# shichaoy/cube_slam

Hardware: AMD Instinct MI355X
Metric: frames/sec front-end (ORB extract + LSD+LBD lines + cuboid: Canny+DT+sweep+score+select) @640x480 (higher is better)
Workload: dtype f64

## Files before the change

### cube_slam_amd/csrc/lsd.hip

```cpp
#include "common.h"
#include "glibc_sincosf.h"
#include "lsd_regions.h"

#include <cfloat>
#include <chrono>
#include <cmath>
#include <mutex>
#include <omp.h>
#include <vector>

namespace {
constexpr double NOTDEF = -1024.0, PI_ = 3.1415926535897932384626433832795, DEG_TO_RADS = PI_ / 180;
constexpr float NOTDEF_DEG = -1024.0f;
constexpr int KH = 3;

__host__ __device__ inline float fast_atan2f_(float y, float x) {
    const float p1 = 0.9997878412794807f * (float)(180 / PI_), p3 = -0.3258083974640975f * (float)(180 / PI_), p5 = 0.1555786518463281f * (float)(180 / PI_),
                p7 = -0.04432655554792128f * (float)(180 / PI_);
    float ax = fabsf(x), ay = fabsf(y), a, c, c2;
    if (ax >= ay) { c = ay / (ax + (float)DBL_EPSILON); c2 = c * c; a = (((p7 * c2 + p5) * c2 + p3) * c2 + p1) * c; }
    else { c = ax / (ay + (float)DBL_EPSILON); c2 = c * c; a = 90.f - (((p7 * c2 + p5) * c2 + p3) * c2 + p1) * c; }
    if (x < 0) a = 180.f - a;
    if (y < 0) a = 360.f - a;
    return a;
// ... 819 lines not shown
    }
    return status;
}

int cs_lsd_read_filter_lines(cs_ctx *ctx, cs_lsd *l, float length_thres, float *lines, int cap, int *counts, int n_frames) {
    if (!ctx || !l || !lines || !counts || cap < 1 || n_frames < 0 || (size_t)n_frames < l->keylines.size()) return CS_ERR_BAD_ARG;
    int status = CS_OK;
    for (size_t f = 0; f < l->keylines.size(); f++) {
        int n = 0;
        for (const cs_keyline &k : l->keylines[f])
            if (k.octave == 0 && k.lineLength > length_thres) {
                if (n < cap) { float *o = lines + (f * cap + n) * 4; o[0] = k.startPointX * 1.f; o[1] = k.startPointY * 1.f; o[2] = k.endPointX * 1.f; o[3] = k.endPointY * 1.f; }
                n++;
            }
        counts[f] = std::min(n, cap);
        if (n > cap) status = CS_ERR_CAPACITY;
    }
    return status;
}

int cs_lsd_upload(cs_ctx *ctx, cs_lsd *l, const uint8_t *gray, int n_frames, int stride) {
    int r = lsd_upload(ctx, l, gray, n_frames, stride); if (r) return r;
    CS_HIP(ctx, hipStreamSynchronize(ctx->stream));
    return CS_OK;
}

int cs_lsd_geometry(const cs_lsd *l, int *width, int *height, int *max_frames) {
    if (!l) return CS_ERR_BAD_ARG;
    *width = l->W; *height = l->H; *max_frames = l->max_frames;
    return CS_OK;
}
int cs_lsd_set_frames_device(cs_ctx *ctx, cs_lsd *l, const uint8_t *d_gray, int n_frames) {
    if (!ctx || !l || !d_gray || n_frames < 1 || n_frames > l->max_frames) return CS_ERR_BAD_ARG;
    CS_HIP(ctx, hipSetDevice(ctx->device));
    l->n_frames = n_frames; l->have_desc = false;
    CS_HIP(ctx, hipMemcpyAsync(l->d_gray, d_gray, (size_t)n_frames * l->W * l->H, hipMemcpyDeviceToDevice, ctx->stream));
    return CS_OK;
}

int cs_lsd_run(cs_ctx *ctx, cs_lsd *l, int with_lbd) { return lsd_run(ctx, l, with_lbd); }

int cs_lsd_set_region_stage(cs_lsd *l, int stage) {
    if (!l || stage < CS_LSD_REGIONS_AUTO || stage > CS_LSD_REGIONS_BACKLOG) return CS_ERR_BAD_ARG;
    l->region_stage = stage;
    return CS_OK;
}

int cs_lsd_region_stats(cs_ctx *ctx, cs_lsd *l, long out[5]) {
    if (!ctx || !l || !out) return CS_ERR_BAD_ARG;
    for (int i = 0; i < 5; i++) out[i] = l->rg_stats[i];
    return CS_OK;
}

int cs_lsd_read(cs_ctx *ctx, cs_lsd *l, int frame, cs_keyline *out, int cap, int *count, uint8_t *desc) {
    if (!ctx || !l || frame < 0 || frame >= l->n_frames || !count || (int)l->keylines.size() <= frame || (desc && !l->have_desc)) return CS_ERR_BAD_ARG;
    const int n = (int)l->keylines[frame].size();
    *count = n;
    if (!out) return CS_OK;
    if (n > cap) return CS_ERR_CAPACITY;
    memcpy(out, l->keylines[frame].data(), sizeof(cs_keyline) * (size_t)n);
    if (desc && n > 0) memcpy(desc, l->h_desc.p + (size_t)l->line_off[frame] * 32, (size_t)n * 32);
    return CS_OK;
}

int cs_lsd_get_maps(cs_ctx *ctx, cs_lsd *l, int frame, double *scaled, double *modgrad, double *angles, int *sw, int *sh) {
    if (!ctx || !l || frame < 0 || frame >= l->n_frames || !sw || !sh) return CS_ERR_BAD_ARG;
    *sw = l->w; *sh = l->h;
    const size_t n = (size_t)l->w * l->h;
    int r;
    if (scaled) {
        if (!l->scaled_kept) { ctx->err = "cs_lsd_get_maps: the scaled frames are only kept for a batch of the host region stage (a device stage takes their buffer over); modgrad and angles are kept"; return CS_ERR_BAD_ARG; }
        r = cs_d2h(ctx, scaled, l->d_scaled + n * frame, n); if (r) return r;
    }
    if (modgrad) { r = cs_d2h(ctx, modgrad, l->d_mod + n * frame, n); if (r) return r; }
    std::vector<float> deg;
    if (angles) { deg.resize(n); r = cs_d2h(ctx, deg.data(), l->d_ang + n * frame, n); if (r) return r; }
    CS_HIP(ctx, hipStreamSynchronize(ctx->stream));
    if (angles) for (size_t i = 0; i < n; i++) angles[i] = deg[i] == NOTDEF_DEG ? NOTDEF : double(deg[i]) * DEG_TO_RADS;
    return CS_OK;
}

}

int cs_lsd_filter_lines_packed(cs_lsd *l, float length_thres, std::vector<int> &offsets, std::vector<double> &lines) {
    if (!l) return CS_ERR_BAD_ARG;
    offsets.assign(l->keylines.size() + 1, 0); lines.clear();
    for (size_t f = 0; f < l->keylines.size(); f++) {
        for (const cs_keyline &k : l->keylines[f])
            if (k.octave == 0 && k.lineLength > length_thres) { lines.push_back((double)(k.startPointX * 1.f)); lines.push_back((double)(k.startPointY * 1.f)); lines.push_back((double)(k.endPointX * 1.f)); lines.push_back((double)(k.endPointY * 1.f)); }
        offsets[f + 1] = (int)(lines.size() / 4);
    }
    if (lines.empty()) lines.push_back(0.0);
    return CS_OK;
}
void cs_lsd_set_gate(cs_lsd *l, void (*wait)(void *), void (*done)(void *), void *arg) { l->gate_wait = wait; l->gate_done = done; l->gate_arg = arg; }
void cs_lsd_set_shared_gpu(cs_lsd *l, int shared) {
    l->seq_wpb = shared ? 4 : 16;
    l->walk_bg = shared != 0;
}
```

### cube_slam_amd/csrc/lsd_regions.h

```cpp
#pragma once
#include <vector>

#include <hip/hip_runtime.h>
struct cs_ctx;
struct LsdSeq;
int lsd_seq_run(cs_ctx *ctx, LsdSeq **handle, int F, int w, int h, const float *d_ang, const double *d_mod, const int *d_caddr, const float *d_cdeg, const float2 *d_ccs, const int *frame_base,
                std::vector<std::vector<float>> &lines, long *stats, void (*before_seq)(void *), void (*after_seq)(void *), void *gate_arg, int grp_p, int waves_per_workgroup = 16, void *scratch = nullptr,
                size_t scratch_bytes = 0, bool pix_ready = false, bool walk_bg = false);
void lsd_seq_destroy(cs_ctx *ctx, LsdSeq *r);
```

### cube_slam_amd/csrc/lsd_regions.hip

```cpp
#include "common.h"

#include <cfloat>
#include <climits>
#include <cmath>
#include <vector>

#include "lsd_regions.h"
#include "lsd_rg_seq.h"
#include "lsd_rg_wlk.h"

namespace {
constexpr int PAD_PX = 272, PAD_LIST = 272, PAD_RECT = 34;
constexpr double PI_ = rg::PI_, LOG_EPS = 0.0, LSD_SCALE = 0.8;
struct AngMap { int w, h; const float *deg; };

__device__ __forceinline__ double rg_log_gamma_windschitl(double x) { return 0.918938533204673 + (x - 0.5) * log(x) - x + 0.5 * x * log(x * sinh(1 / x) + 1 / (810.0 * pow(x, 6.0))); }
__device__ double rg_log_gamma(double x) {
    if (x > 15.0) return rg_log_gamma_windschitl(x);
    const double q[7] = {75122.6331530, 80916.6278952, 36308.2951477, 8687.24529705, 1168.92649479, 83.8676043424, 2.50662827511};
    double a = (x + 0.5) * log(x + 5.5) - (x + 5.5), b = 0;
    for (int n = 0; n < 7; ++n) { a -= log(x + double(n)); b += q[n] * pow(x, double(n)); }
    return a + log(b);
}
#ifndef RG_IMPROVE_WAVES
#ifndef RG_IMPROVE_WAVES
#define RG_IMPROVE_WAVES 3
#endif
#endif
constexpr int LG_N = 32768;
__global__ void __launch_bounds__(256) lsd_rg_lgamma_table(double *t) { const int i = blockIdx.x * 256 + threadIdx.x; if (i < LG_N) t[i] = i > 0 ? rg_log_gamma(double(i)) : 0.0; }
__device__ __forceinline__ double rg_lgam_int(int x, const double *lgt) { return x < LG_N ? lgt[x] : rg_log_gamma_windschitl(double(x)); }
__device__ double rg_nfa(int n, int k, double p, double LOG_NT, const double *lgt) {
    if (n == 0 || k == 0) return -LOG_NT;
    if (n == k) return -LOG_NT - double(n) * log10(p);
    const double p_term = p / (1 - p);
    const double log1term = (double(n) + 1) - rg_lgam_int(k + 1, lgt) - rg_lgam_int(n - k + 1, lgt) + double(k) * log(p) + double(n - k) * log(1.0 - p);
    double term = exp(log1term);
    const double RELATIVE_ERROR_FACTOR = 100.0;
    auto double_equal = [&](double a, double b) { if (a == b) return true; double abs_diff = fabs(a - b), aa = fabs(a), bb = fabs(b); double abs_max = aa > bb ? aa : bb; if (abs_max < DBL_MIN) abs_max = DBL_MIN; return (abs_diff / abs_max) <= (RELATIVE_ERROR_FACTOR * DBL_EPSILON); };
    if (double_equal(term, 0)) { if (k > n * p) return -log1term / 2.30258509299404568402 - LOG_NT; else return -LOG_NT; }
    double bin_tail = term;
    const double tolerance = 0.1;
    for (int i = k + 1; i <= n; ++i) {
        const double bin_term = double(n - i + 1) / double(i), mult_term = bin_term * p_term;
        term *= mult_term;
        bin_tail += term;
        if (bin_term < 1) {
            const double err = term * ((1 - pow(mult_term, double(n - i + 1))) / (1 - mult_term) - 1);
            if (err < tolerance * fabs(-log10(bin_tail) - LOG_NT) * bin_tail) break;
        }
    }
    return -log10(bin_tail) - LOG_NT;
}
struct RectSpan {
    int mnX, lmY, rmY, flstep, slstep, frstep, srstep, y_first, y_hi;
    __device__ __forceinline__ void set(const rg::Rect &rec, int h) {
        const double half_width = rec.width / 2.0, dyhw = rec.dy * half_width, dxhw = rec.dx * half_width;
        int x0 = int(rec.x1 - dyhw), y0 = int(rec.y1 + dxhw), x1 = int(rec.x2 - dyhw), y1 = int(rec.y2 + dxhw);
        int x2 = int(rec.x2 + dyhw), y2 = int(rec.y2 - dxhw), x3 = int(rec.x1 + dyhw), y3 = int(rec.y1 - dxhw);
        auto cswap = [](int &xa, int &ya, int &xb, int &yb) {
            const bool sw = xa > xb || (xa == xb && ya > yb);
            const int tx = sw ? xb : xa, ty = sw ? yb : ya; xb = sw ? xa : xb; yb = sw ? ya : yb; xa = tx; ya = ty;
        };
        cswap(x0, y0, x1, y1); cswap(x2, y2, x3, y3); cswap(x0, y0, x2, y2); cswap(x1, y1, x3, y3); cswap(x1, y1, x2, y2);
        int mnI = 0, mnY = y0; mnX = x0;
        { bool c = mnY > y1; mnI = c ? 1 : mnI; mnX = c ? x1 : mnX; mnY = c ? y1 : mnY; c = mnY > y2; mnI = c ? 2 : mnI; mnX = c ? x2 : mnX; mnY = c ? y2 : mnY; c = mnY > y3; mnI = c ? 3 : mnI; mnX = c ? x3 : mnX; mnY = c ? y3 : mnY; }
        const int mxY = max(max(y0, y1), max(y2, y3));
        const bool m0 = mnI == 0, le1 = mnI <= 1, is3 = mnI == 3;
        const int lmX = m0 ? x1 : x0; lmY = m0 ? y1 : y0;
        const int iX = le1 ? x2 : x1, iY = le1 ? y2 : y1, jX = is3 ? x2 : x3, jY = is3 ? y2 : y3;
        const bool rj = iX < jX;
        const int rmX = rj ? jX : iX, tlX = rj ? iX : jX; rmY = rj ? jY : iY;
        flstep = (mnY != lmY) ? (mnX - lmX) / (mnY - lmY) : 0;
        slstep = (lmY != tlX) ? (lmX - tlX) / (lmY - tlX) : 0;
        frstep = (mnY != rmY) ? (mnX - rmX) / (mnY - rmY) : 0;
        srstep = (rmY != tlX) ? (rmX - tlX) / (rmY - tlX) : 0;
        y_hi = min(mxY, h - 1); y_first = max(mnY, 0);
    }
    __device__ __forceinline__ bool row(int y, int w, int &lx, int &rx) const {
        const long r = (long)y - y_first;
        auto adv = [&](int first, int second, int ysw) -> long {
            long nf = (long)ysw - y_first; if (nf < 0) nf = 0; if (nf > r) nf = r;
            return nf * first + (r - nf) * second;
        };
        const long lxl = max((long)mnX + adv(flstep, slstep, lmY), 0L), rxl = min((long)mnX + adv(frstep, srstep, rmY), (long)w - 1);
        lx = (int)lxl; rx = (int)rxl;
        return rxl >= lxl;
    }
};
template <int NP> __device__ __forceinline__ void rg_row_count(const float *row, int lx, int rx, int g, int G, double theta, const double *precs, int *alg_pts) {
    for (int x = lx + g; x <= rx; x += 4 * G) {
        float ad[4];
#pragma unroll
        for (int u = 0; u < 4; u++) { const int xx = x + u * G; ad[u] = row[xx <= rx ? xx : rx]; }
#pragma unroll
        for (int u = 0; u < 4; u++) {
            const bool in = x + u * G <= rx && ad[u] != rgs::NOTDEF_F;
            const double a = double(ad[u]) * rg::DEG_TO_RADS;
            const double d = fabs(theta - a), d2 = fabs(d - rg::M_2__PI_), nt = d > rg::M_3_2_PI_ ? d2 : d;
            for (int k = 0; k < NP; k++) alg_pts[k] += in && nt <= precs[k];
        }
    }
}
template <int NP> __device__ void rg_rect_count(const AngMap &F, const rg::Rect &rec, const double *precs, int lane, int &total, int *algs) {
    RectSpan S; S.set(rec, F.h);
    int total_pts = 0, alg_pts[NP];
    for (int k = 0; k < NP; k++) alg_pts[k] = 0;
    const int rows = S.y_hi - S.y_first + 1;
    const int G = (rows > 0 && rows < 64) ? 64 / rows : 1, RB = 64 / G;
    const int lrow = lane / G, g = lane - lrow * G;
    for (int yb = S.y_first; yb <= S.y_hi; yb += RB) {
        const int y = yb + lrow;
        int lx, rx;
        if (y > S.y_hi || lrow >= RB || !S.row(y, F.w, lx, rx)) continue;
        if (g == 0) total_pts += rx - lx + 1;
        rg_row_count<NP>(F.deg + (size_t)y * F.w, lx, rx, g, G, rec.theta, precs, alg_pts);
    }
    for (int off = 32; off > 0; off >>= 1) {
        total_pts += __shfl_xor(total_pts, off);
        for (int k = 0; k < NP; k++) alg_pts[k] += __shfl_xor(alg_pts[k], off);
    }
    total = total_pts;
    for (int k = 0; k < NP; k++) algs[k] = alg_pts[k];
}
__device__ __forceinline__ void rg_rect_count_group(const AngMap &F, const rg::Rect &rec, bool on, int sub, int &tot, int &alg) {
    RectSpan S; S.set(rec, F.h);
    int total_pts = 0, alg_pts[1] = {0};
    if (on)
        for (int y = S.y_first + sub; y <= S.y_hi; y += 8) {
            int lx, rx;
            if (!S.row(y, F.w, lx, rx)) continue;
            total_pts += rx - lx + 1;
            rg_row_count<1>(F.deg + (size_t)y * F.w, lx, rx, 0, 1, rec.theta, &rec.prec, alg_pts);
        }
    for (int off = 1; off < 8; off <<= 1) { total_pts += __shfl_xor(total_pts, off); alg_pts[0] += __shfl_xor(alg_pts[0], off); }
    tot = total_pts; alg = alg_pts[0];
}
__device__ __forceinline__ rg::Rect rg_rect_shfl(const rg::Rect &r, int src) {
    rg::Rect o;
    o.x1 = __shfl(r.x1, src); o.y1 = __shfl(r.y1, src); o.x2 = __shfl(r.x2, src); o.y2 = __shfl(r.y2, src); o.width = __shfl(r.width, src); o.x = __shfl(r.x, src);
    o.y = __shfl(r.y, src); o.theta = __shfl(r.theta, src); o.dx = __shfl(r.dx, src); o.dy = __shfl(r.dy, src); o.prec = __shfl(r.prec, src); o.p = __shfl(r.p, src);
    return o;
}
__device__ double rg_rect_improve(const AngMap &F, rg::Rect &rec, double LOG_NT, int lane, const double *lgt, double log_nfa) {
    const double delta = 0.5, delta_2 = delta / 2.0;
    if (log_nfa > LOG_EPS) return log_nfa;
    const int g = lane >> 3, sub = lane & 7;
    rg::Rect mine;
    int tot = 0, al = 0, cnt = 0;
    auto tolerances = [&]() {
        mine = rec;
        double p = rec.p, precs[5];
#pragma unroll
        for (int n = 0; n < 5; ++n) { p /= 2; precs[n] = p * PI_; if (n <= g) { mine.p = p; mine.prec = precs[n]; } }
        int t, alg[5]; rg_rect_count<5>(F, rec, precs, lane, t, alg);
        tot = t; al = alg[0];
#pragma unroll
        for (int n = 1; n < 5; ++n) if (g == n) al = alg[n];
        cnt = 5;
    };
    auto shrink = [&](int side) {
        mine = rec; cnt = 0;
        double wd = rec.width;
#pragma unroll
        for (int n = 0; n < 5; ++n) if ((wd - delta) >= 0.5) { wd -= delta; cnt++; }
#pragma unroll
        for (int n = 0; n < 5; ++n) if (n <= g && (mine.width - delta) >= 0.5) {
            if (side == 1) { mine.x1 += -mine.dy * delta_2; mine.y1 += mine.dx * delta_2; mine.x2 += -mine.dy * delta_2; mine.y2 += mine.dx * delta_2; }
            else if (side == 2) { mine.x1 -= -mine.dy * delta_2; mine.y1 -= mine.dx * delta_2; mine.x2 -= -mine.dy * delta_2; mine.y2 -= mine.dx * delta_2; }
            mine.width -= delta;
        }
        if (cnt) rg_rect_count_group(F, mine, g < cnt, sub, tot, al);
    };
    auto take_best = [&]() {
        const bool on = g < cnt;
        const double mv = rg_nfa(on ? tot : 0, on ? al : 0, mine.p, LOG_NT, lgt);
        int best = -1;
#pragma unroll
        for (int n = 0; n < 5; ++n) { const double vn = __shfl(mv, 8 * n); if (n < cnt && vn > log_nfa) { log_nfa = vn; best = n; } }
        if (best >= 0) rec = rg_rect_shfl(mine, 8 * best);
    };
    tolerances(); take_best();
    if (log_nfa > LOG_EPS) return log_nfa;
    for (int side = 0; side < 3; side++) {
        shrink(side);
        if (cnt) take_best();
        if (log_nfa > LOG_EPS) return log_nfa;
    }
    if ((rec.width - delta) >= 0.5) { tolerances(); take_best(); }
    return log_nfa;
}

struct SeqParams {
    int F, w, h;
    const int *caddr; const int *frame_base; const float *cdeg; const float2 *ccs; const double *mod; const float *ang;
    float *ang32; float *seed_cs; int *glist; double *rect; size_t rect_stride; int cand_cap; int *cand_cnt; int *status;
    int min_reg_size, list_cap;
    size_t pix_stride;
};
__global__ void __launch_bounds__(256) lsd_rg_fill32(float4 *ang, size_t n4) {
    const size_t i = (size_t)blockIdx.x * 256 + threadIdx.x;
    if (i < n4) ang[i] = make_float4(rgs::NOTDEF_F, rgs::NOTDEF_F, rgs::NOTDEF_F, rgs::NOTDEF_F);
}
__global__ void __launch_bounds__(256) lsd_rg_scatter(SeqParams P) {
    const int f = blockIdx.y, base = P.frame_base[f], ne = P.frame_base[f + 1] - base;
    const int i = blockIdx.x * 256 + threadIdx.x;
    if (i >= ne) return;
    const int q = P.caddr[base + i] & 0x7fffffff;
    const float d = P.cdeg[base + i];
    P.ang32[(size_t)f * P.pix_stride + q] = d;
    const double a = double(d) * rg::DEG_TO_RADS;
    reinterpret_cast<float2 *>(P.seed_cs)[base + i] = make_float2(float(cos(a)), float(sin(a)));
}
__device__ __forceinline__ void lsd_rg_seq_body(const SeqParams &P) {
    const int f = __builtin_amdgcn_readfirstlane(blockIdx.x * (blockDim.x >> 6) + (threadIdx.x >> 6));
    if (f >= P.F) return;
#ifdef RGS_PRIO
    __builtin_amdgcn_s_setprio(RGS_PRIO);
#endif
    const int base = P.frame_base[f];
    rgs::Frame Fr;
    Fr.w = P.w; Fr.h = P.h; Fr.ne = P.frame_base[f + 1] - base;
    Fr.caddr = P.caddr + base; Fr.fre = P.ang32 + (size_t)f * P.pix_stride; Fr.ang = P.ang + (size_t)f * P.w * P.h; Fr.mod = P.mod + (size_t)f * P.w * P.h; Fr.seed_cs = P.seed_cs + 2 * (size_t)base;
    Fr.rect = P.rect + (size_t)f * P.rect_stride; Fr.cand_cap = P.cand_cap; Fr.cand_cnt = P.cand_cnt + f;
    Fr.status = P.status + 4 * f; Fr.min_reg_size = P.min_reg_size; Fr.list_cap = P.list_cap;
    rgs::List L;
    L.glob = P.glist + (size_t)f * rgs::CAP; L.ring[0] = 0;
    rgs::run_frame<rgs::Wave>(Fr, L);
}
#ifdef RGS_WAVES
__global__ void __launch_bounds__(1024) __attribute__((amdgpu_waves_per_eu(RGS_WAVES, RGS_WAVES))) lsd_rg_seq(SeqParams P) { lsd_rg_seq_body(P); }
#else
__global__ void __launch_bounds__(1024) lsd_rg_seq(SeqParams P) { lsd_rg_seq_body(P); }
#endif
constexpr int WLK_SLICES = 8;
struct WlkLaunch { rgl::Batch slice[WLK_SLICES]; int n_slices, waves_per_slice; };
template <int NS> struct WlkMail {
    rgw::Mail<NS> &m; int base;
    __device__ __forceinline__ rgw::Mail<NS> &mail() { return m; }
    __device__ __forceinline__ int slot_of(int l) const { return base + l; }
    __device__ __forceinline__ int ring_size() const { return NS; }
    __device__ __forceinline__ void after_iteration(const rgl::Batch &) {}
};
template <int WK, int NWAVES, int ACC> __global__ void __launch_bounds__(64 * NWAVES) lsd_rg_wlk(WlkLaunch L, int blocks_per_slice) {
    constexpr int NS = WK * 64;
    __shared__ rgw::Mail<NS> mail;
    for (int k = threadIdx.x; k < NS; k += 64 * NWAVES) { mail.slot[k].state = 0; mail.slot[k].fl = 0; mail.ring_id[k] = 0; mail.ring_tick[k] = 0; }
    if (threadIdx.x == 0) { mail.tail = 0; mail.head = 0; mail.walkers_done = 0; }
    __syncthreads();
    const int wv = __builtin_amdgcn_readfirstlane(threadIdx.x >> 6), lane = threadIdx.x & 63;
    const int c = blockIdx.x / blocks_per_slice;
    const rgl::Batch &B = L.slice[c];
    if (wv < WK) {
        const int f0 = ((blockIdx.x - c * blocks_per_slice) * WK + wv) * 64;
        if (f0 < B.F) { WlkMail<NS> mp{mail, wv * 64}; rgw::run_walker<rgl::LWave, ACC>(B, f0, mp); }
        rgw::wg_release();
        if (lane == 0) rgw::lds_add(&mail.walkers_done, 1);
        return;
    }
    for (;;) {
        int t = 0;
        if (lane == 0) t = rgw::lds_add(&mail.head, 1);
        t = __builtin_amdgcn_readfirstlane(t);
        bool quit = false;
        while (__builtin_amdgcn_readfirstlane(rgw::lds_ld(&mail.ring_tick[t % NS])) != t + 1) {
            if (__builtin_amdgcn_readfirstlane(rgw::lds_ld(&mail.walkers_done)) == WK && __builtin_amdgcn_readfirstlane(rgw::lds_ld(&mail.tail)) <= t) { quit = true; break; }
            __builtin_amdgcn_s_sleep(4);
        }
        if (quit) break;
        rgw::serve_ticket<rgs::Wave, NS>(B, mail, t);
    }
}
__global__ void __launch_bounds__(1024) lsd_rg_cand_scan(const int *cand_cnt, int F, int *cand_base) {
    __shared__ int part[1024];
    const int t = threadIdx.x, per = (F + 1023) / 1024;
    int sum = 0;
    for (int k = 0; k < per; k++) { const int f = t * per + k; if (f < F) sum += cand_cnt[f]; }
    part[t] = sum;
    __syncthreads();
    for (int d = 1; d < 1024; d <<= 1) { const int v = t >= d ? part[t - d] : 0; __syncthreads(); part[t] += v; __syncthreads(); }
    int run = part[t] - sum;
    for (int k = 0; k < per; k++) { const int f = t * per + k; if (f < F) { cand_base[f] = run; run += cand_cnt[f]; } }
    if (t == 1023) cand_base[F] = part[1023];
}
__global__ void __launch_bounds__(256) __attribute__((amdgpu_waves_per_eu(RG_IMPROVE_WAVES, RG_IMPROVE_WAVES))) lsd_rg_improve(SeqParams P, const int *cand_base, int n_cand, const double *lgt, float4 *line, uint8_t *has) {
    const int base = (blockIdx.x * 4 + (threadIdx.x >> 6)) * 8, lane = threadIdx.x & 63, grp = lane >> 3, sub = lane & 7;
    if (base >= n_cand) return;
    const double LOG_NT = 5 * (log10(double(P.w)) + log10(double(P.h))) / 2 + log10(11.0);
    auto frame_of = [&](int wv) { int lo = 0, hi = P.F; while (hi - lo > 1) { const int mid = (lo + hi) >> 1; if (cand_base[mid] <= wv) lo = mid; else hi = mid; } return lo; };
    auto load_rect = [&](int wv, int f, rg::Rect &rec) {
        const double *o = P.rect + (size_t)f * P.rect_stride + (size_t)(wv - cand_base[f]) * 12;
        rec.x1 = o[0]; rec.y1 = o[1]; rec.x2 = o[2]; rec.y2 = o[3]; rec.width = o[4]; rec.x = o[5]; rec.y = o[6]; rec.theta = o[7]; rec.dx = o[8]; rec.dy = o[9]; rec.prec = o[10]; rec.p = o[11];
    };
    auto emit = [&](int wv, rg::Rect rec, double log_nfa) {
        const bool ok = log_nfa > LOG_EPS;
        if (ok) {
            rec.x1 += 0.5; rec.y1 += 0.5; rec.x2 += 0.5; rec.y2 += 0.5;
            rec.x1 /= LSD_SCALE; rec.y1 /= LSD_SCALE; rec.x2 /= LSD_SCALE; rec.y2 /= LSD_SCALE;
            line[wv] = make_float4(float(rec.x1), float(rec.y1), float(rec.x2), float(rec.y2));
        }
        has[wv] = ok ? 1 : 0;
    };
    const int mine = base + grp;
    const bool on = mine < n_cand;
    const int f1 = frame_of(on ? mine : n_cand - 1);
    rg::Rect r1;
    load_rect(on ? mine : n_cand - 1, f1, r1);
    double log1;
    {
        RectSpan S; S.set(r1, P.h);
        const float *deg = P.ang + (size_t)f1 * P.w * P.h;
        int tot = 0, alg[1] = {0};
        if (on)
            for (int y = S.y_first + sub; y <= S.y_hi; y += 8) {
                int lx, rx;
                if (!S.row(y, P.w, lx, rx)) continue;
                tot += rx - lx + 1;
                rg_row_count<1>(deg + (size_t)y * P.w, lx, rx, 0, 1, r1.theta, &r1.prec, alg);
            }
        for (int off = 1; off < 8; off <<= 1) { tot += __shfl_xor(tot, off); alg[0] += __shfl_xor(alg[0], off); }
        log1 = rg_nfa(tot, alg[0], r1.p, LOG_NT, lgt);
    }
    if (on && sub == 0 && log1 > LOG_EPS) emit(mine, r1, log1);
    unsigned long long todo = __ballot(on && sub == 0 && !(log1 > LOG_EPS));
    while (todo) {
        const int l = __ffsll((long long)todo) - 1;
        todo &= todo - 1;
        const int wv = base + (l >> 3), f = __shfl(f1, l);
        const double first = __shfl(log1, l);
        rg::Rect rec;
        load_rect(wv, f, rec);
        const AngMap Fr = {P.w, P.h, P.ang + (size_t)f * P.w * P.h};
        const double log_nfa = rg_rect_improve(Fr, rec, LOG_NT, lane, lgt, first);
        if (lane == 0) emit(wv, rec, log_nfa);
    }
}
}

struct LsdSeq {
    int F = 0, w = 0, h = 0; int cand_cap = 0; size_t cap_lines = 0;
    float *d_pix = nullptr; bool pix_borrowed = false;
    rgl::Ent *d_elist = nullptr; float *d_ang32 = nullptr; int *d_order = nullptr;
    int *d_glist = nullptr, *d_cand_cnt = nullptr, *d_cand_base = nullptr, *d_status = nullptr, *d_frame_base = nullptr;
    double *d_rect = nullptr, *d_lgt = nullptr;
    uint8_t *d_has = nullptr;
    float4 *d_line = nullptr;
    cs_pinned<int> h_base, h_status; cs_pinned<uint8_t> h_has; cs_pinned<float4> h_line;
};
void lsd_seq_destroy(cs_ctx *ctx, LsdSeq *r) {
    if (!r) return;
    void *ptrs[] = {r->d_elist, r->d_ang32, r->d_order, r->pix_borrowed ? nullptr : r->d_pix, r->d_glist, r->d_cand_cnt, r->d_cand_base, r->d_status, r->d_frame_base, r->d_rect, r->d_lgt, r->d_has, r->d_line};
    for (void *p : ptrs) cs_dfree(ctx, p);
    r->h_base.release(); r->h_status.release(); r->h_has.release(); r->h_line.release();
    delete r;
}
int lsd_seq_run(cs_ctx *ctx, LsdSeq **handle, int F, int w, int h, const float *d_ang, const double *d_mod, const int *d_caddr, const float *d_cdeg, const float2 *d_ccs, const int *frame_base,
                std::vector<std::vector<float>> &lines, long *stats ,
                void (*before_seq)(void *), void (*after_seq)(void *), void *gate_arg ,
                int grp_p ,
                int waves_per_workgroup ,
                void *scratch, size_t scratch_bytes ,
                bool pix_ready ,
                bool walk_bg ) {
    LsdSeq *r = *handle;
    if (w > 0xffff || h > 0x7fff) return CS_ERR_CAPACITY;
    int max_ne = 0;
    for (int f = 0; f < F; f++) max_ne = std::max(max_ne, frame_base[f + 1] - frame_base[f]);
    int rc;
#define RA_(call) do { rc = (call); if (rc != CS_OK) return rc; } while (0)
    if (!r || r->F < F || r->w != w || r->h != h) {
        lsd_seq_destroy(ctx, r);
        r = new LsdSeq();
        *handle = r;
        r->F = F; r->w = w; r->h = h; r->cand_cap = 4096;
        RA_(cs_dalloc(ctx, &r->d_order, (size_t)F)); RA_(cs_dalloc(ctx, &r->d_rect, (size_t)F * (r->cand_cap * 12 + PAD_RECT)));
        RA_(cs_dalloc(ctx, &r->d_cand_cnt, (size_t)F)); RA_(cs_dalloc(ctx, &r->d_cand_base, (size_t)F + 1));
        RA_(cs_dalloc(ctx, &r->d_status, (size_t)F * 4)); RA_(cs_dalloc(ctx, &r->d_frame_base, (size_t)F + 1));
        RA_(cs_dalloc(ctx, &r->d_lgt, (size_t)LG_N));
        CS_LAUNCH(ctx, "lsd_rg_lgamma_table", lsd_rg_lgamma_table, dim3(LG_N / 256), dim3(256), 0, r->d_lgt);
    }
    RA_(cs_h2d(ctx, r->d_frame_base, frame_base, (size_t)F + 1));
    SeqParams S;
    S.F = F; S.w = w; S.h = h; S.caddr = d_caddr; S.frame_base = r->d_frame_base; S.cdeg = d_cdeg; S.ccs = d_ccs; S.mod = d_mod; S.ang = d_ang;
    S.ang32 = nullptr; S.seed_cs = reinterpret_cast<float *>(const_cast<float2 *>(d_ccs));  S.glist = r->d_glist; S.rect = r->d_rect; S.cand_cap = r->cand_cap; S.cand_cnt = r->d_cand_cnt; S.status = r->d_status;
    const double LOG_NT = 5 * (std::log10(double(w)) + std::log10(double(h))) / 2 + std::log10(11.0);
    S.min_reg_size = int(-LOG_NT / std::log10(rg::ANG_TH / 180));
    S.list_cap = rgs::CAP;
    if (const char *e = getenv("CUBESLAM_LSD_SEQ_CAP")) S.list_cap = std::max(2, std::min(rgs::CAP, atoi(e)));
    if (grp_p != 0 && grp_p != 65) return CS_ERR_BAD_ARG;
    const bool grp = grp_p == 65, pad = grp;
    const size_t rect_stride = (size_t)r->cand_cap * 12 + (pad ? PAD_RECT : 0), list_stride = (size_t)rgl::CAP + (pad ? PAD_LIST : 0);
    S.pix_stride = (size_t)w * h + (pad ? PAD_PX : 0); S.rect_stride = rect_stride;
    const size_t npx = (size_t)F * S.pix_stride;
    if (grp) {
        const size_t head = (size_t)((w + 8 + 3) & ~3);
        if (!r->d_ang32) RA_(cs_dalloc(ctx, &r->d_ang32, head + (size_t)r->F * ((size_t)w * h + PAD_PX) + 16));
        if (!r->d_elist) RA_(cs_dalloc(ctx, &r->d_elist, (size_t)r->F * ((size_t)rgl::CAP + PAD_LIST) + 16));
        S.ang32 = r->d_ang32 + head;
        CS_LAUNCH(ctx, "lsd_rg_fill", lsd_rg_fill32, dim3((unsigned)(((npx + head) / 4 + 1 + 255) / 256)), dim3(256), 0, reinterpret_cast<float4 *>(r->d_ang32), (npx + head) / 4 + 1);
    } else {
        if (!r->d_pix) {
            if (scratch && scratch_bytes >= (size_t)r->F * w * h * sizeof(float) + 64) { r->d_pix = static_cast<float *>(scratch); r->pix_borrowed = true; }
            else RA_(cs_dalloc(ctx, &r->d_pix, (size_t)r->F * w * h + 16));
        }
        if (!r->d_glist) RA_(cs_dalloc(ctx, &r->d_glist, (size_t)r->F * rgs::CAP));
        S.ang32 = r->d_pix; S.glist = r->d_glist;
        if (pix_ready && !r->pix_borrowed) { ctx->err = "lsd_seq_run: the pixel records were announced in the scratch buffer, but the stage does not use it for this batch"; return CS_ERR_BAD_ARG; }
        if (!pix_ready) CS_LAUNCH(ctx, "lsd_rg_fill", lsd_rg_fill32, dim3((unsigned)((npx / 4 + 1 + 255) / 256)), dim3(256), 0, reinterpret_cast<float4 *>(r->d_pix), npx / 4 + 1);
    }
    if (!pix_ready) CS_LAUNCH(ctx, "lsd_rg_scatter", lsd_rg_scatter, dim3((max_ne + 255) / 256, F), dim3(256), 0, S);
    int wpb = std::max(1, std::min(16, waves_per_workgroup));
    RA_(r->h_base.reserve(ctx, (size_t)F + 1)); RA_(r->h_status.reserve(ctx, (size_t)F * 4));
    if (before_seq) before_seq(gate_arg);
    if (grp) {
        const size_t npx = (size_t)w * h, head = (size_t)((w + 8 + 3) & ~3);
        int chunk = (int)std::min<size_t>(4096, 0xffffffffull / (npx * sizeof(double)));
        chunk = std::min(chunk, 1024);
        if (chunk < 1) return CS_ERR_CAPACITY;
        std::vector<int> order((size_t)F);
        for (int c0 = 0; c0 < F; c0 += chunk) {
            const int fc = std::min(chunk, F - c0);
            for (int k = 0; k < fc; k++) order[(size_t)c0 + k] = k;
            std::stable_sort(order.begin() + c0, order.begin() + c0 + fc, [&](int a, int b) { return frame_base[c0 + a + 1] - frame_base[c0 + a] > frame_base[c0 + b + 1] - frame_base[c0 + b]; });
        }
        RA_(cs_h2d(ctx, r->d_order, order.data(), (size_t)F));
        CS_HIP(ctx, hipStreamSynchronize(ctx->stream));
        for (int l0 = 0; l0 < F; l0 += chunk * WLK_SLICES) {
            WlkLaunch L;
            L.n_slices = 0; L.waves_per_slice = (chunk + 63) / 64;
            for (int c0 = l0; c0 < F && L.n_slices < WLK_SLICES; c0 += chunk) {
                const int fc = std::min(chunk, F - c0);
                rgl::Batch &B = L.slice[L.n_slices++];
                B.F = fc; B.w = w; B.h = h; B.npx = (int)npx; B.order = r->d_order + c0; B.ang_stride = (int)S.pix_stride; B.list_stride = (int)list_stride; B.rect_stride = (int)rect_stride; B.ang_head = (int)head;
                B.caddr = d_caddr + frame_base[c0]; B.frame_base = r->d_frame_base + c0; B.ang = r->d_ang32 + (size_t)c0 * S.pix_stride; B.mod = d_mod + (size_t)c0 * npx; B.seed_cs = S.seed_cs + 2 * (size_t)frame_base[c0];
                B.list = r->d_elist + (size_t)c0 * list_stride; B.list_cap = std::min(S.list_cap, rgl::CAP); B.rect = r->d_rect + (size_t)c0 * rect_stride; B.cand_cap = r->cand_cap; B.cand_cnt = r->d_cand_cnt + c0; B.status = r->d_status + 4 * (size_t)c0;
                B.min_reg_size = S.min_reg_size; B.max_iters = (int)std::min<size_t>(64 * npx, 0x7fffffff);
            }
            int wk = 1, nw = 8, acc = 1;
            if (const char *e = getenv("CUBESLAM_LSD_WLK")) sscanf(e, "%d,%d,%d", &wk, &nw, &acc);
            const int bps = (L.waves_per_slice + wk - 1) / wk, groups = L.n_slices * bps;
#define WLK_(WK, NW, AC) else if (wk == WK && nw == NW && acc == AC) CS_LAUNCH(ctx, "lsd_rg_wlk", (lsd_rg_wlk<WK, NW, AC>), dim3(groups), dim3(64 * NW), 0, L, bps)
            if (false) {}
            WLK_(1, 8, 1); WLK_(1, 8, 2); WLK_(2, 8, 1); WLK_(8, 16, 1);
            else { ctx->err = "CUBESLAM_LSD_WLK: no such shape (walkers,waves,accepts)"; return CS_ERR_BAD_ARG; }
#undef WLK_
        }
    } else if (walk_bg) {
        CS_HIP(ctx, ctx->bg_begin());
        CS_LAUNCH_BG(ctx, "lsd_rg_seq", lsd_rg_seq, dim3((F + wpb - 1) / wpb), dim3(64 * wpb), 0, S);
        CS_LAUNCH_BG(ctx, "lsd_rg_cand_scan", lsd_rg_cand_scan, dim3(1), dim3(1024), 0, r->d_cand_cnt, F, r->d_cand_base);
        CS_HIP(ctx, hipMemcpyAsync(r->h_base.p, r->d_cand_base, ((size_t)F + 1) * sizeof(int), hipMemcpyDeviceToHost, ctx->bg_stream));
        CS_HIP(ctx, hipMemcpyAsync(r->h_status.p, r->d_status, (size_t)F * 4 * sizeof(int), hipMemcpyDeviceToHost, ctx->bg_stream));
        CS_HIP(ctx, ctx->bg_end());
    } else
    CS_LAUNCH(ctx, "lsd_rg_seq", lsd_rg_seq, dim3((F + wpb - 1) / wpb), dim3(64 * wpb), 0, S);
    if (grp || !walk_bg) {
        CS_LAUNCH(ctx, "lsd_rg_cand_scan", lsd_rg_cand_scan, dim3(1), dim3(1024), 0, r->d_cand_cnt, F, r->d_cand_base);
        RA_(cs_d2h(ctx, r->h_base.p, r->d_cand_base, (size_t)F + 1));
        RA_(cs_d2h(ctx, r->h_status.p, r->d_status, (size_t)F * 4));
        CS_HIP(ctx, hipStreamSynchronize(ctx->stream));
    }
    if (after_seq) after_seq(gate_arg);
    long grows = 0, fetches = 0, nreg = 0;
    bool bad = false;
    for (int f = 0; f < F; f++) { grows += r->h_status.p[4 * f]; bad = bad || r->h_status.p[4 * f + 1] != 0; nreg += r->h_status.p[4 * f + 2]; fetches += r->h_status.p[4 * f + 3]; }
    const int n_cand = r->h_base.p[F];
    if (stats) { stats[0] = grows; stats[1] = fetches; stats[2] = n_cand; stats[3] = nreg; }
    if (bad) return CS_ERR_CAPACITY;
    lines.assign((size_t)F, {});
    if (n_cand == 0) return CS_OK;
    if ((size_t)n_cand > r->cap_lines) {
        cs_dfree(ctx, r->d_line); cs_dfree(ctx, r->d_has);
        r->d_line = nullptr; r->d_has = nullptr; r->cap_lines = 0;
        const size_t cap = (size_t)n_cand + n_cand / 4 + 1024;
        RA_(cs_dalloc(ctx, &r->d_line, cap)); RA_(cs_dalloc(ctx, &r->d_has, cap));
        r->cap_lines = cap;
    }
    CS_LAUNCH(ctx, "lsd_rg_improve", lsd_rg_improve, dim3((n_cand + 31) / 32), dim3(256), 0, S, r->d_cand_base, n_cand, r->d_lgt, r->d_line, r->d_has);
    RA_(r->h_has.reserve(ctx, (size_t)n_cand)); RA_(r->h_line.reserve(ctx, (size_t)n_cand));
    RA_(cs_d2h(ctx, r->h_has.p, r->d_has, (size_t)n_cand));
    RA_(cs_d2h(ctx, r->h_line.p, r->d_line, (size_t)n_cand));
    CS_HIP(ctx, hipStreamSynchronize(ctx->stream));
#undef RA_
#pragma omp parallel for schedule(static) num_threads(std::max(1, std::min(ctx->host_threads, F)))
    for (int f = 0; f < F; f++)
        for (int k = r->h_base.p[f]; k < r->h_base.p[f + 1]; k++)
            if (r->h_has.p[k]) { const float4 v = r->h_line.p[k]; lines[f].push_back(v.x); lines[f].push_back(v.y); lines[f].push_back(v.z); lines[f].push_back(v.w); }
    return CS_OK;
}
```

### cube_slam_amd/lsd.py

```python
import ctypes as C

import numpy as np

from . import _lib
from ._lib import Handle, check, lib, ptr

KEYLINE_DTYPE = np.dtype([("angle", "f4"), ("class_id", "i4"), ("octave", "i4"), ("pt", "f4", 2), ("response", "f4"), ("size", "f4"),
                          ("startPointX", "f4"), ("startPointY", "f4"), ("endPointX", "f4"), ("endPointY", "f4"),
                          ("sPointInOctaveX", "f4"), ("sPointInOctaveY", "f4"), ("ePointInOctaveX", "f4"), ("ePointInOctaveY", "f4"),
                          ("lineLength", "f4"), ("numOfPixels", "i4")])


class line_lbd_detect(Handle):
    HANDLE, DESTROY = "_l", "cs_lsd_destroy"

    def __init__(self, width, height, max_frames=1, ctx=None, device=0):
        self.ctx = ctx or _lib.Context(device)
        self.use_LSD = True
        self.line_length_thres = 50.0
        self.W, self.H, self.max_frames = width, height, max_frames
        self.cap = 8192
        self._l = C.c_void_p()
        check(self.ctx.ptr, lib().cs_lsd_create(self.ctx.ptr, width, height, max_frames, C.byref(self._l)), "cs_lsd_create")

    def _imgs(self, gray):
        g = np.ascontiguousarray(gray, np.uint8)
        if g.ndim == 2:
            g = g[None]
        assert g.shape[1:] == (self.H, self.W) and len(g) <= self.max_frames
        return g

    def upload(self, gray):
        g = self._imgs(gray)
        self._n = len(g)
        check(self.ctx.ptr, lib().cs_lsd_upload(self.ctx.ptr, self._l, ptr(g), len(g), self.W), "cs_lsd_upload")

    def run(self, with_lbd=True):
        check(self.ctx.ptr, lib().cs_lsd_run(self.ctx.ptr, self._l, int(with_lbd)), "cs_lsd_run")

    def set_region_stage(self, stage):
        check(self.ctx.ptr, lib().cs_lsd_set_region_stage(self._l, {"auto": 0, "host": 1, "wave_per_frame": 2, "backlog": 3}[stage]), "cs_lsd_set_region_stage")

    def region_stats(self):
        st = (C.c_long * 5)()
        check(self.ctx.ptr, lib().cs_lsd_region_stats(self.ctx.ptr, self._l, st), "cs_lsd_region_stats")
        return {"device": bool(st[0]), "grows": st[1], "candidates": st[2], "host_fallback": bool(st[3]), "fetches": st[4]}

    def read(self, frame, with_desc=True):
        n = C.c_int()
        check(self.ctx.ptr, lib().cs_lsd_read(self.ctx.ptr, self._l, frame, None, 0, C.byref(n), None), "cs_lsd_read")
        kl = np.zeros(n.value, KEYLINE_DTYPE); desc = np.zeros((n.value, 32), np.uint8)
        check(self.ctx.ptr, lib().cs_lsd_read(self.ctx.ptr, self._l, frame, ptr(kl), n.value, C.byref(n), ptr(desc) if with_desc else None), "cs_lsd_read")
        return (kl, desc) if with_desc else kl

    def read_filter_lines(self, n_frames, cap=1024):
        out = np.zeros((n_frames, cap, 4), np.float32); counts = np.zeros(n_frames, np.int32)
        check(self.ctx.ptr, lib().cs_lsd_read_filter_lines(self.ctx.ptr, self._l, self.line_length_thres, ptr(out), cap, ptr(counts), int(n_frames)), "cs_lsd_read_filter_lines")
        return [out[f, :counts[f]] for f in range(n_frames)]

    def detect_raw_lines(self, gray):
        g = self._imgs(gray)
        out = np.zeros((len(g), self.cap), KEYLINE_DTYPE); counts = np.zeros(len(g), np.int32)
        check(self.ctx.ptr, lib().cs_lsd_detect(self.ctx.ptr, self._l, ptr(g), len(g), self.W, ptr(out), self.cap, ptr(counts)), "cs_lsd_detect")
        res = [out[f, :counts[f]].copy() for f in range(len(g))]
        return res if np.ndim(gray) == 3 else res[0]

    def detect_filter_lines(self, gray):
        g = self._imgs(gray)
        out = np.zeros((len(g), self.cap, 4), np.float32); counts = np.zeros(len(g), np.int32)
        check(self.ctx.ptr, lib().cs_lsd_detect_filter_lines(self.ctx.ptr, self._l, ptr(g), len(g), self.W, self.line_length_thres, ptr(out),
                                                             self.cap, ptr(counts)), "cs_lsd_detect_filter_lines")
        res = [out[f, :counts[f]].copy() for f in range(len(g))]
        return res if np.ndim(gray) == 3 else res[0]

    def maps(self, frame=0):
        sw, sh = C.c_int(), C.c_int()
        check(self.ctx.ptr, lib().cs_lsd_get_maps(self.ctx.ptr, self._l, frame, None, None, None, C.byref(sw), C.byref(sh)), "cs_lsd_get_maps")
        n = sw.value * sh.value
        sc, mg, an = np.zeros(n), np.zeros(n), np.zeros(n)
        check(self.ctx.ptr, lib().cs_lsd_get_maps(self.ctx.ptr, self._l, frame, ptr(sc), ptr(mg), ptr(an), C.byref(sw), C.byref(sh)), "cs_lsd_get_maps")
        shape = (sh.value, sw.value)
        return sc.reshape(shape), mg.reshape(shape), an.reshape(shape)

    def get_line_descriptors(self, gray, keylines, want_float=False):
        g = np.ascontiguousarray(gray, np.uint8)
        kl = np.ascontiguousarray(keylines, KEYLINE_DTYPE); n = len(kl)
        desc = np.zeros((n, 32), np.uint8); fd = np.zeros((n, 72), np.float32) if want_float else None
        check(self.ctx.ptr, lib().cs_lbd_compute(self.ctx.ptr, ptr(g), g.shape[1], g.shape[0], g.shape[1], ptr(kl), n,
                                                 ptr(desc), ptr(fd) if want_float else None), "cs_lbd_compute")
        return (desc, fd) if want_float else desc

    def detect_descrip_lines(self, gray):
        kl = self.detect_raw_lines(gray)
        desc = self.get_line_descriptors(gray, kl)
        keep = (kl["octave"] == 0) & (kl["lineLength"] > self.line_length_thres)
        return kl[keep], desc[keep]

    def match_line_descrip(self, desc_q, desc_t, matching_dist_thres=25.0):
        q = np.ascontiguousarray(desc_q, np.uint8).reshape(-1, 32); t = np.ascontiguousarray(desc_t, np.uint8).reshape(-1, 32)
# ... 10 lines not shown
```

Before: 28420.

## Precompute LSD NFA table and look it up in rect improve, deferring misses

Builds a device table of NFA values for n up to 511, all k, and eleven power-of-two probabilities, computed once at setup. The main rect-improve kernel looks NFA values up from this table instead of evaluating the log-gamma binomial tail, and scores the five tolerance variants with a grouped count path. Candidates whose parameters fall outside the table are marked deferred and recomputed exactly by a second kernel. This adds a table-build launch, an extra kernel pass and a counter readback, plus a probe API for checking table accuracy.

```diff
diff --git a/cube_slam_amd/csrc/lsd.hip b/cube_slam_amd/csrc/lsd.hip
--- a/cube_slam_amd/csrc/lsd.hip
+++ b/cube_slam_amd/csrc/lsd.hip
@@ -895,6 +895,12 @@
     return CS_OK;
 }
 
+int cs_lsd_nfa_probe(cs_ctx *ctx, cs_lsd *l, int m, const int *triples, double *out, long *counters) {
+    if (!ctx || !l) return CS_ERR_BAD_ARG;
+    CS_HIP(ctx, hipSetDevice(ctx->device));
+    return lsd_seq_nfa_probe(ctx, l->seq, m, triples, out, counters);
+}
+
 int cs_lsd_read(cs_ctx *ctx, cs_lsd *l, int frame, cs_keyline *out, int cap, int *count, uint8_t *desc) {
     if (!ctx || !l || frame < 0 || frame >= l->n_frames || !count || (int)l->keylines.size() <= frame || (desc && !l->have_desc)) return CS_ERR_BAD_ARG;
     const int n = (int)l->keylines[frame].size();
diff --git a/cube_slam_amd/csrc/lsd_regions.h b/cube_slam_amd/csrc/lsd_regions.h
--- a/cube_slam_amd/csrc/lsd_regions.h
+++ b/cube_slam_amd/csrc/lsd_regions.h
@@ -8,3 +8,4 @@
                 std::vector<std::vector<float>> &lines, long *stats, void (*before_seq)(void *), void (*after_seq)(void *), void *gate_arg, int grp_p, int waves_per_workgroup = 16, void *scratch = nullptr,
                 size_t scratch_bytes = 0, bool pix_ready = false, bool walk_bg = false);
 void lsd_seq_destroy(cs_ctx *ctx, LsdSeq *r);
+int lsd_seq_nfa_probe(cs_ctx *ctx, LsdSeq *r, int m, const int *triples, double *out, long *counters);
diff --git a/cube_slam_amd/csrc/lsd_regions.hip b/cube_slam_amd/csrc/lsd_regions.hip
--- a/cube_slam_amd/csrc/lsd_regions.hip
+++ b/cube_slam_amd/csrc/lsd_regions.hip
@@ -52,6 +52,32 @@
     }
     return -log10(bin_tail) - LOG_NT;
 }
+__device__ __forceinline__ double rg_log_nt(int w, int h) { return 5 * (log10(double(w)) + log10(double(h))) / 2 + log10(11.0); }
+constexpr int NFA_NP = 11, NFA_NMAX = 511, NFA_TRI = (NFA_NMAX + 1) * (NFA_NMAX + 2) / 2;
+__global__ void __launch_bounds__(256) lsd_rg_nfa_table(double *T, int w, int h, const double *lgt) {
+    const int i = blockIdx.x * 256 + threadIdx.x, j = blockIdx.y;
+    if (i >= NFA_TRI) return;
+    int n = int((sqrt(8.0 * i + 1) - 1) / 2);
+    while (n * (n + 1) / 2 > i) n--;
+    while ((n + 1) * (n + 2) / 2 <= i) n++;
+    T[(size_t)j * NFA_TRI + i] = rg_nfa(n, i - n * (n + 1) / 2, ldexp(1.0, -(3 + j)), rg_log_nt(w, h), lgt);
+}
+struct NfaDirect {
+    static constexpr bool GROUP_TOLERANCES = false;
+    double LOG_NT; const double *lgt;
+    __device__ __forceinline__ double operator()(int n, int k, double p, bool &) const { return rg_nfa(n, k, p, LOG_NT, lgt); }
+};
+struct NfaTable {
+    static constexpr bool GROUP_TOLERANCES = true;
+    const double *T; int nmax;
+    __device__ __forceinline__ double operator()(int n, int k, double p, bool &miss) const {
+        const long long b = __double_as_longlong(p);
+        const int j = 1020 - int(b >> 52);
+        const bool ok = (b & 0xfffffffffffffLL) == 0 && j >= 0 && j < NFA_NP && n <= nmax && k >= 0 && k <= n;
+        miss = !ok;
+        return T[ok ? (size_t)j * NFA_TRI + n * (n + 1) / 2 + k : 0];
+    }
+};
 struct RectSpan {
     int mnX, lmY, rmY, flstep, slstep, frstep, srstep, y_first, y_hi;
     __device__ __forceinline__ void set(const rg::Rect &rec, int h) {
@@ -142,7 +168,7 @@
     o.y = __shfl(r.y, src); o.theta = __shfl(r.theta, src); o.dx = __shfl(r.dx, src); o.dy = __shfl(r.dy, src); o.prec = __shfl(r.prec, src); o.p = __shfl(r.p, src);
     return o;
 }
-__device__ double rg_rect_improve(const AngMap &F, rg::Rect &rec, double LOG_NT, int lane, const double *lgt, double log_nfa) {
+template <class E> __device__ double rg_rect_improve(const AngMap &F, rg::Rect &rec, const E &nfa, int lane, double log_nfa, bool &missed) {
     const double delta = 0.5, delta_2 = delta / 2.0;
     if (log_nfa > LOG_EPS) return log_nfa;
     const int g = lane >> 3, sub = lane & 7;
@@ -153,11 +179,12 @@
         double p = rec.p, precs[5];
 #pragma unroll
         for (int n = 0; n < 5; ++n) { p /= 2; precs[n] = p * PI_; if (n <= g) { mine.p = p; mine.prec = precs[n]; } }
+        cnt = 5;
+        if constexpr (E::GROUP_TOLERANCES) { rg_rect_count_group(F, mine, g < 5, sub, tot, al); return; }
         int t, alg[5]; rg_rect_count<5>(F, rec, precs, lane, t, alg);
         tot = t; al = alg[0];
 #pragma unroll
         for (int n = 1; n < 5; ++n) if (g == n) al = alg[n];
-        cnt = 5;
     };
     auto shrink = [&](int side) {
         mine = rec; cnt = 0;
@@ -174,18 +201,20 @@
     };
     auto take_best = [&]() {
         const bool on = g < cnt;
-        const double mv = rg_nfa(on ? tot : 0, on ? al : 0, mine.p, LOG_NT, lgt);
+        bool miss = false;
+        const double mv = nfa(on ? tot : 0, on ? al : 0, mine.p, miss);
+        if (__any(on && miss)) { missed = true; return; }
         int best = -1;
 #pragma unroll
         for (int n = 0; n < 5; ++n) { const double vn = __shfl(mv, 8 * n); if (n < cnt && vn > log_nfa) { log_nfa = vn; best = n; } }
         if (best >= 0) rec = rg_rect_shfl(mine, 8 * best);
     };
     tolerances(); take_best();
-    if (log_nfa > LOG_EPS) return log_nfa;
+    if (missed || log_nfa > LOG_EPS) return log_nfa;
     for (int side = 0; side < 3; side++) {
         shrink(side);
         if (cnt) take_best();
-        if (log_nfa > LOG_EPS) return log_nfa;
+        if (missed || log_nfa > LOG_EPS) return log_nfa;
     }
     if ((rec.width - delta) >= 0.5) { tolerances(); take_best(); }
     return log_nfa;
@@ -283,10 +312,16 @@
     for (int k = 0; k < per; k++) { const int f = t * per + k; if (f < F) { cand_base[f] = run; run += cand_cnt[f]; } }
     if (t == 1023) cand_base[F] = part[1023];
 }
-__global__ void __launch_bounds__(256) __attribute__((amdgpu_waves_per_eu(RG_IMPROVE_WAVES, RG_IMPROVE_WAVES))) lsd_rg_improve(SeqParams P, const int *cand_base, int n_cand, const double *lgt, float4 *line, uint8_t *has) {
+constexpr uint8_t HAS_DEFERRED = 2;
+template <class E, bool REDO> __device__ __forceinline__ void lsd_rg_improve_body(const SeqParams &P, const int *cand_base, int n_cand, const E &nfa, float4 *line, uint8_t *has, unsigned long long *counters) {
     const int base = (blockIdx.x * 4 + (threadIdx.x >> 6)) * 8, lane = threadIdx.x & 63, grp = lane >> 3, sub = lane & 7;
     if (base >= n_cand) return;
-    const double LOG_NT = 5 * (log10(double(P.w)) + log10(double(P.h))) / 2 + log10(11.0);
+    const int mine = base + grp;
+    bool on = mine < n_cand;
+    if (REDO) {
+        on = on && has[mine] == HAS_DEFERRED;
+        if (!__any(on)) return;
+    }
     auto frame_of = [&](int wv) { int lo = 0, hi = P.F; while (hi - lo > 1) { const int mid = (lo + hi) >> 1; if (cand_base[mid] <= wv) lo = mid; else hi = mid; } return lo; };
     auto load_rect = [&](int wv, int f, rg::Rect &rec) {
         const double *o = P.rect + (size_t)f * P.rect_stride + (size_t)(wv - cand_base[f]) * 12;
@@ -301,12 +336,11 @@
         }
         has[wv] = ok ? 1 : 0;
     };
-    const int mine = base + grp;
-    const bool on = mine < n_cand;
     const int f1 = frame_of(on ? mine : n_cand - 1);
     rg::Rect r1;
     load_rect(on ? mine : n_cand - 1, f1, r1);
     double log1;
+    bool miss1 = false;
     {
         RectSpan S; S.set(r1, P.h);
         const float *deg = P.ang + (size_t)f1 * P.w * P.h;
@@ -319,10 +353,11 @@
                 rg_row_count<1>(deg + (size_t)y * P.w, lx, rx, 0, 1, r1.theta, &r1.prec, alg);
             }
         for (int off = 1; off < 8; off <<= 1) { tot += __shfl_xor(tot, off); alg[0] += __shfl_xor(alg[0], off); }
-        log1 = rg_nfa(tot, alg[0], r1.p, LOG_NT, lgt);
-    }
-    if (on && sub == 0 && log1 > LOG_EPS) emit(mine, r1, log1);
-    unsigned long long todo = __ballot(on && sub == 0 && !(log1 > LOG_EPS));
+        log1 = nfa(tot, alg[0], r1.p, miss1);
+    }
+    if (on && sub == 0) { if (miss1) has[mine] = HAS_DEFERRED; else if (log1 > LOG_EPS) emit(mine, r1, log1); }
+    int n_deferred = __popcll(__ballot(on && sub == 0 && miss1));
+    unsigned long long todo = __ballot(on && sub == 0 && !miss1 && !(log1 > LOG_EPS));
     while (todo) {
         const int l = __ffsll((long long)todo) - 1;
         todo &= todo - 1;
@@ -331,9 +366,28 @@
         rg::Rect rec;
         load_rect(wv, f, rec);
         const AngMap Fr = {P.w, P.h, P.ang + (size_t)f * P.w * P.h};
-        const double log_nfa = rg_rect_improve(Fr, rec, LOG_NT, lane, lgt, first);
-        if (lane == 0) emit(wv, rec, log_nfa);
-    }
+        bool missed = false;
+        const double log_nfa = rg_rect_improve(Fr, rec, nfa, lane, first, missed);
+        if (missed) { n_deferred++; if (lane == 0) has[wv] = HAS_DEFERRED; }
+        else if (lane == 0) emit(wv, rec, log_nfa);
+    }
+    if (!REDO && lane == 0) atomicAdd(counters, (unsigned long long)(min(8, n_cand - base) - n_deferred) | (unsigned long long)n_deferred << 32);
+}
+__global__ void __launch_bounds__(256) __attribute__((amdgpu_waves_per_eu(4, 4))) lsd_rg_improve(SeqParams P, const int *cand_base, int n_cand, const double *nfa_table, int nfa_nmax, float4 *line, uint8_t *has, unsigned long long *counters) {
+    lsd_rg_improve_body<NfaTable, false>(P, cand_base, n_cand, NfaTable{nfa_table, nfa_nmax}, line, has, counters);
+}
+__global__ void __launch_bounds__(256) __attribute__((amdgpu_waves_per_eu(RG_IMPROVE_WAVES, RG_IMPROVE_WAVES))) lsd_rg_improve_deferred(SeqParams P, const int *cand_base, int n_cand, const double *lgt, float4 *line, uint8_t *has) {
+    lsd_rg_improve_body<NfaDirect, true>(P, cand_base, n_cand, NfaDirect{rg_log_nt(P.w, P.h), lgt}, line, has, nullptr);
+}
+__global__ void __launch_bounds__(256) lsd_rg_nfa_probe(const int *t, int m, const double *nfa_table, int nfa_nmax, int w, int h, const double *lgt, double *out) {
+    const int i = blockIdx.x * 256 + threadIdx.x;
+    if (i >= m) return;
+    const int n = t[3 * i], k = t[3 * i + 1], j = t[3 * i + 2];
+    const double p = ldexp(1.0, -(3 + j));
+    bool miss = false;
+    const double v = NfaTable{nfa_table, nfa_nmax}(n, k, p, miss);
+    out[2 * i] = miss ? __longlong_as_double(0x7ff8000000000000LL) : v;
+    out[2 * i + 1] = rg_nfa(n, k, p, rg_log_nt(w, h), lgt);
 }
 }
 
@@ -342,16 +396,21 @@
     float *d_pix = nullptr; bool pix_borrowed = false;
     rgl::Ent *d_elist = nullptr; float *d_ang32 = nullptr; int *d_order = nullptr;
     int *d_glist = nullptr, *d_cand_cnt = nullptr, *d_cand_base = nullptr, *d_status = nullptr, *d_frame_base = nullptr;
-    double *d_rect = nullptr, *d_lgt = nullptr;
+    double *d_rect = nullptr, *d_lgt = nullptr, *d_nfa = nullptr;
+    unsigned long long *d_counters = nullptr; cs_pinned<unsigned long long> h_counters; long nfa_counts[2] = {0, 0};
     uint8_t *d_has = nullptr;
     float4 *d_line = nullptr;
     cs_pinned<int> h_base, h_status; cs_pinned<uint8_t> h_has; cs_pinned<float4> h_line;
 };
+static int lsd_nfa_bound() {
+    const char *e = getenv("CUBESLAM_LSD_NFA_NMAX");
+    return e ? std::max(0, std::min(NFA_NMAX, atoi(e))) : NFA_NMAX;
+}
 void lsd_seq_destroy(cs_ctx *ctx, LsdSeq *r) {
     if (!r) return;
-    void *ptrs[] = {r->d_elist, r->d_ang32, r->d_order, r->pix_borrowed ? nullptr : r->d_pix, r->d_glist, r->d_cand_cnt, r->d_cand_base, r->d_status, r->d_frame_base, r->d_rect, r->d_lgt, r->d_has, r->d_line};
+    void *ptrs[] = {r->d_elist, r->d_ang32, r->d_order, r->pix_borrowed ? nullptr : r->d_pix, r->d_glist, r->d_cand_cnt, r->d_cand_base, r->d_status, r->d_frame_base, r->d_rect, r->d_lgt, r->d_nfa, r->d_counters, r->d_has, r->d_line};
     for (void *p : ptrs) cs_dfree(ctx, p);
-    r->h_base.release(); r->h_status.release(); r->h_has.release(); r->h_line.release();
+    r->h_base.release(); r->h_status.release(); r->h_has.release(); r->h_line.release(); r->h_counters.release();
     delete r;
 }
 int lsd_seq_run(cs_ctx *ctx, LsdSeq **handle, int F, int w, int h, const float *d_ang, const double *d_mod, const int *d_caddr, const float *d_cdeg, const float2 *d_ccs, const int *frame_base,
@@ -378,6 +437,8 @@
         RA_(cs_dalloc(ctx, &r->d_status, (size_t)F * 4)); RA_(cs_dalloc(ctx, &r->d_frame_base, (size_t)F + 1));
         RA_(cs_dalloc(ctx, &r->d_lgt, (size_t)LG_N));
         CS_LAUNCH(ctx, "lsd_rg_lgamma_table", lsd_rg_lgamma_table, dim3(LG_N / 256), dim3(256), 0, r->d_lgt);
+        RA_(cs_dalloc(ctx, &r->d_nfa, (size_t)NFA_NP * NFA_TRI)); RA_(cs_dalloc(ctx, &r->d_counters, (size_t)1)); RA_(r->h_counters.reserve(ctx, (size_t)1));
+        CS_LAUNCH(ctx, "lsd_rg_nfa_table", lsd_rg_nfa_table, dim3((NFA_TRI + 255) / 256, NFA_NP), dim3(256), 0, r->d_nfa, w, h, r->d_lgt);
     }
     RA_(cs_h2d(ctx, r->d_frame_base, frame_base, (size_t)F + 1));
     SeqParams S;
@@ -387,6 +448,7 @@
     S.min_reg_size = int(-LOG_NT / std::log10(rg::ANG_TH / 180));
     S.list_cap = rgs::CAP;
     if (const char *e = getenv("CUBESLAM_LSD_SEQ_CAP")) S.list_cap = std::max(2, std::min(rgs::CAP, atoi(e)));
+    const int nfa_nmax = lsd_nfa_bound();
     if (grp_p != 0 && grp_p != 65) return CS_ERR_BAD_ARG;
     const bool grp = grp_p == 65, pad = grp;
     const size_t rect_stride = (size_t)r->cand_cap * 12 + (pad ? PAD_RECT : 0), list_stride = (size_t)rgl::CAP + (pad ? PAD_LIST : 0);
@@ -468,6 +530,7 @@
     if (stats) { stats[0] = grows; stats[1] = fetches; stats[2] = n_cand; stats[3] = nreg; }
     if (bad) return CS_ERR_CAPACITY;
     lines.assign((size_t)F, {});
+    r->nfa_counts[0] = r->nfa_counts[1] = 0;
     if (n_cand == 0) return CS_OK;
     if ((size_t)n_cand > r->cap_lines) {
         cs_dfree(ctx, r->d_line); cs_dfree(ctx, r->d_has);
@@ -476,11 +539,15 @@
         RA_(cs_dalloc(ctx, &r->d_line, cap)); RA_(cs_dalloc(ctx, &r->d_has, cap));
         r->cap_lines = cap;
     }
-    CS_LAUNCH(ctx, "lsd_rg_improve", lsd_rg_improve, dim3((n_cand + 31) / 32), dim3(256), 0, S, r->d_cand_base, n_cand, r->d_lgt, r->d_line, r->d_has);
     RA_(r->h_has.reserve(ctx, (size_t)n_cand)); RA_(r->h_line.reserve(ctx, (size_t)n_cand));
+    CS_HIP(ctx, hipMemsetAsync(r->d_counters, 0, sizeof(unsigned long long), ctx->stream));
+    CS_LAUNCH(ctx, "lsd_rg_improve", lsd_rg_improve, dim3((n_cand + 31) / 32), dim3(256), 0, S, r->d_cand_base, n_cand, r->d_nfa, nfa_nmax ? nfa_nmax : -1, r->d_line, r->d_has, r->d_counters);
+    CS_LAUNCH(ctx, "lsd_rg_improve_deferred", lsd_rg_improve_deferred, dim3((n_cand + 31) / 32), dim3(256), 0, S, r->d_cand_base, n_cand, r->d_lgt, r->d_line, r->d_has);
     RA_(cs_d2h(ctx, r->h_has.p, r->d_has, (size_t)n_cand));
     RA_(cs_d2h(ctx, r->h_line.p, r->d_line, (size_t)n_cand));
+    RA_(cs_d2h(ctx, r->h_counters.p, r->d_counters, (size_t)1));
     CS_HIP(ctx, hipStreamSynchronize(ctx->stream));
+    r->nfa_counts[0] = (long)(r->h_counters.p[0] & 0xffffffffull); r->nfa_counts[1] = (long)(r->h_counters.p[0] >> 32);
 #undef RA_
 #pragma omp parallel for schedule(static) num_threads(std::max(1, std::min(ctx->host_threads, F)))
     for (int f = 0; f < F; f++)
@@ -488,3 +555,17 @@
             if (r->h_has.p[k]) { const float4 v = r->h_line.p[k]; lines[f].push_back(v.x); lines[f].push_back(v.y); lines[f].push_back(v.z); lines[f].push_back(v.w); }
     return CS_OK;
 }
+int lsd_seq_nfa_probe(cs_ctx *ctx, LsdSeq *r, int m, const int *triples, double *out, long *counters) {
+    if (!r || !r->d_nfa || m < 0 || (m > 0 && (!triples || !out))) return CS_ERR_BAD_ARG;
+    for (int i = 0; i < m; i++) if (triples[3 * i] < 0 || triples[3 * i + 1] < 0 || triples[3 * i + 1] > triples[3 * i] || triples[3 * i + 2] < 0 || triples[3 * i + 2] >= NFA_NP) return CS_ERR_BAD_ARG;
+    if (counters) { counters[0] = r->nfa_counts[0]; counters[1] = r->nfa_counts[1]; }
+    if (m == 0) return CS_OK;
+    const int nfa_nmax = lsd_nfa_bound();
+    cs_scratch tmp(ctx);
+    int *d_t = nullptr; double *d_o = nullptr;
+    CS_TRY(tmp.upload(ctx, &d_t, triples, (size_t)3 * m));
+    CS_TRY(tmp.alloc(ctx, &d_o, (size_t)2 * m));
+    CS_LAUNCH(ctx, "lsd_rg_nfa_probe", lsd_rg_nfa_probe, dim3((m + 255) / 256), dim3(256), 0, d_t, m, r->d_nfa, nfa_nmax ? nfa_nmax : -1, r->w, r->h, r->d_lgt, d_o);
+    CS_TRY(cs_d2h(ctx, out, d_o, (size_t)2 * m));
+    return tmp.drain();
+}
diff --git a/cube_slam_amd/lsd.py b/cube_slam_amd/lsd.py
--- a/cube_slam_amd/lsd.py
+++ b/cube_slam_amd/lsd.py
@@ -45,6 +45,12 @@
         st = (C.c_long * 5)()
         check(self.ctx.ptr, lib().cs_lsd_region_stats(self.ctx.ptr, self._l, st), "cs_lsd_region_stats")
         return {"device": bool(st[0]), "grows": st[1], "candidates": st[2], "host_fallback": bool(st[3]), "fetches": st[4]}
+
+    def nfa_probe(self, triples):
+        t = np.ascontiguousarray(triples, np.int32).reshape(-1, 3)
+        out = np.zeros((len(t), 2), np.float64); cnt = (C.c_long * 2)()
+        check(self.ctx.ptr, lib().cs_lsd_nfa_probe(self.ctx.ptr, self._l, C.c_int(len(t)), ptr(t), ptr(out), cnt), "cs_lsd_nfa_probe")
+        return out[:, 0].copy(), out[:, 1].copy(), cnt[0], cnt[1]
 
     def read(self, frame, with_desc=True):
         n = C.c_int()
```

Measured after the change: 29270, median of 6. 3.0% higher.
